# rhmes/point-cloud-compression

Hardware: AMD Instinct MI355X
Metric: points/sec compress+decompress (ModelNet40-shaped 8192 K=256) (higher is better)
Workload: dtype f32 (operands split into two scaled fp16 pieces of 22-23 bits together, three fp16-MFMA products per fp32 product, fp32 accumulate); 1 GPU; IPDAE K=256 d=16 L=7, 8192-pt CAD-like synthetic clouds (configs[1]); distinct_clouds_per_gpu=1024, points_per_cloud=8192, patches_per_cloud=64, octree_mode=reference, weights=seeded random, matmul=f16x2

## Files before the change

### point-cloud-compression_amd/csrc/rangecoder.hip

```cpp
#include "common.h"
#include "split_stream.h"
#include "entry_index.h"

struct BitWriter {
    uint8_t *buf;
    int cap, n;
    unsigned cache;
    int count;
    __device__ void bit(int b)
    {
        cache = (cache << 1) | (unsigned)(b & 1);
        if (++count == 8) {
            if (n < cap) buf[n] = (uint8_t)cache;
            ++n;
            count = 0; cache = 0;
        }
    }
    __device__ void bit_pending(int b, unsigned long long &pending)
    {
        bit(b);
        while (pending > 0) { bit(!b); --pending; }
    }
    __device__ void flush()
    {
        if (count > 0) {
            cache <<= (8 - count);
            if (n < cap) buf[n] = (uint8_t)cache;
            ++n;
            count = 0; cache = 0;
        }
    }
};

__device__ __forceinline__ int rc_row_bytes(int count, int stride) { return count < 0 ? 0 : (count > stride ? stride : count); }

__device__ __forceinline__ void rc_record(uint32_t *entry, unsigned low, unsigned high, unsigned long long bits, bool pending)
{
    entry[0] = low;
    entry[1] = high;
    entry[2] = (unsigned)(bits < 0x7FFFFFFFull ? bits : 0x7FFFFFFFull) | (pending ? PCCX_INDEX_FLAG : 0u);
}
__device__ __forceinline__ void rc_index_header(uint32_t *index, int nsym, int seg_sym)
{
    index[0] = 0x31495850u;
    index[1] = (unsigned)nsym;
    index[2] = (unsigned)seg_sym;
    index[3] = (unsigned)pccx_index_segments(nsym, seg_sym);
}

template <bool REC>
__device__ __forceinline__ void rc_encode_lane(const int32_t *__restrict__ cdf_int, const float *__restrict__ latent_q, int B, int nsym,
                                               int Lp, int sym_offset, uint8_t *__restrict__ out, int cap, int32_t *__restrict__ nbytes,
                                               int seg_sym, uint8_t *__restrict__ index, int idx_stride,
                                               const int32_t *__restrict__ nsym_of = nullptr)
{
    const int b = blockIdx.x * blockDim.x + threadIdx.x;
    if (b >= B) return;
    const int row = nsym;
    if (nsym_of) nsym = rc_row_bytes(nsym_of[b], row);
    uint32_t *entry = nullptr;
    if (REC) {
        entry = (uint32_t *)(index + (size_t)b * idx_stride);
        rc_index_header(entry, nsym, seg_sym);
        entry += PCCX_INDEX_HEADER_BYTES / 4;
    }
    BitWriter w{out + (size_t)b * cap, cap, 0, 0u, 0};
    unsigned low = 0u, high = 0xFFFFFFFFu;
    unsigned long long pending = 0;
    const int max_symbol = Lp - 2;
    const int32_t *c = cdf_int + (size_t)b * row * Lp;
    const float *q = latent_q + (size_t)b * row;
    int i = 0, stop = REC ? 0 : nsym;
    do {
    if (REC && i < nsym) {
        rc_record(entry, low, high, (unsigned long long)w.n * 8ull + (unsigned long long)w.count + pending, pending > 0);
        entry += PCCX_INDEX_ENTRY_BYTES / 4;
        stop = nsym - i < seg_sym ? nsym : i + seg_sym;
    }
    for (; i < stop; ++i, c += Lp) {
        int s = (int)q[i] + sym_offset;
        s = s < 0 ? 0 : (s > max_symbol ? max_symbol : s);
        const unsigned long long span = (unsigned long long)high - (unsigned long long)low + 1ull;
        const unsigned c_low = (unsigned)c[s] & 0xFFFFu;
        const unsigned c_high = s == max_symbol ? 0x10000u : ((unsigned)c[s + 1] & 0xFFFFu);
        high = (unsigned)((low - 1u) + (unsigned)((span * c_high) >> 16));
        low = (unsigned)(low + (unsigned)((span * c_low) >> 16));
        for (;;) {
            if (high < 0x80000000u) {
                w.bit_pending(0, pending);
                low <<= 1; high <<= 1; high |= 1u;
            } else if (low >= 0x80000000u) {
                w.bit_pending(1, pending);
                low <<= 1; high <<= 1; high |= 1u;
            } else if (low >= 0x40000000u && high < 0xC0000000u) {
                ++pending;
                low <<= 1; low &= 0x7FFFFFFFu;
                high <<= 1; high |= 0x80000001u;
            } else
                break;
        }
    }
    } while (REC && i < nsym);
    ++pending;
    if (low < 0x40000000u) w.bit_pending(0, pending);
    else w.bit_pending(1, pending);
    w.flush();
    nbytes[b] = w.n <= cap ? w.n : -w.n;
}

__global__ void range_encode_kernel(const int32_t *__restrict__ cdf_int, const float *__restrict__ latent_q, int B, int nsym,
                                    int Lp, int sym_offset, uint8_t *__restrict__ out, int cap, int32_t *__restrict__ nbytes)
{
    rc_encode_lane<false>(cdf_int, latent_q, B, nsym, Lp, sym_offset, out, cap, nbytes, 0, nullptr, 0);
}

__global__ void range_encode_indexed_kernel(const int32_t *__restrict__ cdf_int, const float *__restrict__ latent_q, int B, int nsym,
                                            int Lp, int sym_offset, uint8_t *__restrict__ out, int cap, int32_t *__restrict__ nbytes,
                                            int seg_sym, uint8_t *__restrict__ index, int idx_stride)
{
    rc_encode_lane<true>(cdf_int, latent_q, B, nsym, Lp, sym_offset, out, cap, nbytes, seg_sym, index, idx_stride);
}

template <bool REC>
__device__ __forceinline__ void rc_decode_lane(const int32_t *__restrict__ cdf_int, const uint8_t *__restrict__ in, int stride,
                                               const int32_t *__restrict__ nbytes, int B, int nsym, int Lp, int sym_offset,
                                               float *__restrict__ latent_q, int seg_sym, uint8_t *__restrict__ index, int idx_stride,
                                               const int32_t *__restrict__ nsym_of = nullptr)
{
    const int b = blockIdx.x * blockDim.x + threadIdx.x;
    if (b >= B) return;
    const int row = nsym;
    if (nsym_of) {
        nsym = rc_row_bytes(nsym_of[b], row);
        for (int i = nsym; i < row; ++i) latent_q[(size_t)b * row + i] = 0.f;
    }
    uint32_t *entry = nullptr;
    int next = 0;
    unsigned long long shifted = 0;
    bool under = false;
    if (REC) {
        entry = (uint32_t *)(index + (size_t)b * idx_stride);
        rc_index_header(entry, nsym, seg_sym);
        entry += PCCX_INDEX_HEADER_BYTES / 4;
    }
    const uint8_t *buf = in + (size_t)b * stride;
    const int nb = rc_row_bytes(nbytes[b], stride);
    int pos = 0, cached = 0;
    unsigned cache = 0;
    unsigned low = 0u, high = 0xFFFFFFFFu, value = 0u;
    auto get = [&]() {
        if (cached == 0) {
            if (pos >= nb) { value <<= 1; return; }
            cache = buf[pos++]; cached = 8;
        }
        value = (value << 1) | ((cache >> (cached - 1)) & 1u);
        --cached;
    };
    for (int i = 0; i < 32; ++i) get();
    const int max_symbol = Lp - 2;
    const int32_t *c = cdf_int + (size_t)b * row * Lp;
    for (int i = 0; i < nsym; ++i, c += Lp) {
        if (REC && i == next) {
            rc_record(entry, low, high, shifted, under);
            entry += PCCX_INDEX_ENTRY_BYTES / 4;
            next += seg_sym;
        }
        const unsigned long long span = (unsigned long long)high - (unsigned long long)low + 1ull;
        const unsigned count =
            (unsigned)((((unsigned long long)value - (unsigned long long)low + 1ull) * 0x10000ull - 1ull) / span) & 0xFFFFu;
        int left = 0, right = max_symbol + 1;
        while (left + 1 < right) {
            const int mid = (left + right) >> 1;
            if (((unsigned)c[mid] & 0xFFFFu) <= count) left = mid; else right = mid;
        }
        const int s = left;
        if (!REC || latent_q) latent_q[(size_t)b * row + i] = (float)(s - sym_offset);
        const unsigned c_low = (unsigned)c[s] & 0xFFFFu;
        const unsigned c_high = s == max_symbol ? 0x10000u : ((unsigned)c[s + 1] & 0xFFFFu);
        high = (unsigned)((low - 1u) + (unsigned)((span * c_high) >> 16));
        low = (unsigned)(low + (unsigned)((span * c_low) >> 16));
        for (;;) {
            if (low >= 0x80000000u || high < 0x80000000u) {
                low <<= 1; high <<= 1; high |= 1u; get();
                if (REC) ++shifted, under = false;
            } else if (low >= 0x40000000u && high < 0xC0000000u) {
                low <<= 1; low &= 0x7FFFFFFFu;
                high <<= 1; high |= 0x80000001u;
                value -= 0x40000000u;
                get();
                if (REC) ++shifted, under = true;
            } else
                break;
        }
    }
}

__global__ void range_decode_kernel(const int32_t *__restrict__ cdf_int, const uint8_t *__restrict__ in, int stride,
                                    const int32_t *__restrict__ nbytes, int B, int nsym, int Lp, int sym_offset,
                                    float *__restrict__ latent_q)
{
    rc_decode_lane<false>(cdf_int, in, stride, nbytes, B, nsym, Lp, sym_offset, latent_q, 0, nullptr, 0);
}

__global__ void range_index_build_kernel(const int32_t *__restrict__ cdf_int, const uint8_t *__restrict__ in, int stride,
                                         const int32_t *__restrict__ nbytes, int B, int nsym, int Lp, int sym_offset,
                                         float *__restrict__ latent_q, int seg_sym, uint8_t *__restrict__ index, int idx_stride)
{
    rc_decode_lane<true>(cdf_int, in, stride, nbytes, B, nsym, Lp, sym_offset, latent_q, seg_sym, index, idx_stride);
}

__global__ void range_encode_n_kernel(const int32_t *__restrict__ cdf_int, const float *__restrict__ latent_q, int B, int row,
                                      const int32_t *__restrict__ nsym_of, int Lp, int sym_offset, uint8_t *__restrict__ out, int cap,
                                      int32_t *__restrict__ nbytes)
{
    rc_encode_lane<false>(cdf_int, latent_q, B, row, Lp, sym_offset, out, cap, nbytes, 0, nullptr, 0, nsym_of);
}

__global__ void range_decode_n_kernel(const int32_t *__restrict__ cdf_int, const uint8_t *__restrict__ in, int stride,
                                      const int32_t *__restrict__ nbytes, int B, int row, const int32_t *__restrict__ nsym_of, int Lp,
                                      int sym_offset, float *__restrict__ latent_q)
{
    rc_decode_lane<false>(cdf_int, in, stride, nbytes, B, row, Lp, sym_offset, latent_q, 0, nullptr, 0, nsym_of);
}

#define RC_MAX_LDS_BYTES (60 * 1024)

__device__ __forceinline__ unsigned ones(int m) { return m >= 32 ? 0xFFFFFFFFu : ((1u << m) - 1u); }
__device__ __forceinline__ unsigned rc_uni(unsigned v) { return __builtin_amdgcn_readfirstlane(v); }
__device__ __forceinline__ unsigned rc_scale(unsigned span32, unsigned c) { return (unsigned)(((unsigned long long)span32 * c + c) >> 16); }

template <bool REC = false>
__device__ __forceinline__ void rc_encode_wave(unsigned char *smem, const int32_t *__restrict__ c, const float *__restrict__ q, int nsym,
                                               int Lp, int sym_offset, uint8_t *__restrict__ out, int cap, int32_t *__restrict__ nbytes,
                                               uint32_t *__restrict__ entry = nullptr, int seg_sym = 0)
{
    uint2 *sc = (uint2 *)smem;
    unsigned *sout = (unsigned *)(sc + nsym);
    const int lane = threadIdx.x;
    const int capw = (cap + 3) >> 2;
    const int max_symbol = Lp - 2;
    for (int i = lane; i < nsym; i += 64) {
        int s = (int)q[i] + sym_offset;
        s = s < 0 ? 0 : (s > max_symbol ? max_symbol : s);
        const int32_t *ci = c + (size_t)i * Lp;
        sc[i] = make_uint2((unsigned)ci[s] & 0xFFFFu, s == max_symbol ? 0x10000u : ((unsigned)ci[s + 1] & 0xFFFFu));
    }
    __syncthreads();
    unsigned low = 0u, high = 0xFFFFFFFFu;
    unsigned long long pending = 0, acc = 0;
    int na = 0, nw = 0;
    auto put = [&](unsigned v, int cnt) {
        acc = (acc << cnt) | (unsigned long long)v;
        na += cnt;
        if (na >= 32) {
            const unsigned w = (unsigned)(acc >> (na - 32));
            if (nw < capw && lane == 0) sout[nw] = __builtin_bswap32(w);
            ++nw;
            na -= 32;
        }
    };
    auto run = [&](int bit, unsigned long long cnt) {
        while (cnt > 0) {
            const int m = cnt > 32 ? 32 : (int)cnt;
            put(bit ? ones(m) : 0u, m);
            cnt -= m;
        }
    };
    int next = 0;
    uint2 nxt = lane < nsym ? sc[lane] : make_uint2(0u, 0x10000u);
    for (int i0 = 0; i0 < nsym; i0 += 64) {
        const uint2 cur = nxt;
        if (i0 + 64 + lane < nsym) nxt = sc[i0 + 64 + lane];
        const int cnt = nsym - i0 < 64 ? nsym - i0 : 64;
        for (int j = 0; j < cnt; ++j) {
            if (REC && i0 + j == next) {
                if (lane == 0) rc_record(entry, low, high, (unsigned long long)nw * 32ull + (unsigned long long)na + pending, pending > 0);
                entry += PCCX_INDEX_ENTRY_BYTES / 4;
                next += seg_sym;
            }
            const unsigned c_low = __builtin_amdgcn_readlane(cur.x, j), c_high = __builtin_amdgcn_readlane(cur.y, j);
            const unsigned span32 = high - low;
            high = (low - 1u) + rc_scale(span32, c_high);
            low = low + rc_scale(span32, c_low);
            const unsigned x = low ^ high;
            const int m = (int)x < 0 ? 0 : (x ? __clz(x) : 32);
            if (m > 0) {
                const unsigned top = (unsigned)(((unsigned long long)low << m) >> 32);
                if (pending == 0)
                    put(top, m);
                else {
                    const unsigned b0 = low >> 31;
                    put(b0, 1);
                    run(!b0, pending);
                    pending = 0;
                    if (m > 1) put(top & ones(m - 1), m - 1);
                }
                low = (unsigned)((unsigned long long)low << m);
                high = (unsigned)(((unsigned long long)high << m) | (unsigned long long)ones(m));
            }
            const unsigned t = (~low | high) << 1;
            const int k = t ? __clz(t) : 31;
            const unsigned fix = k ? 0x80000000u : 0u;
            low = (low << k) & ~fix;
            high = (high << k) | fix | ones(k);
            pending += k;
        }
    }
    ++pending;
    const int fb = low < 0x40000000u ? 0 : 1;
    put(fb, 1);
    run(!fb, pending);
    int n = nw * 4 + ((na + 7) >> 3);
    if (na > 0 && nw < capw && lane == 0) sout[nw] = __builtin_bswap32((unsigned)(acc << (32 - na)));
    if (lane == 0) *nbytes = n <= cap ? n : -n;
    __syncthreads();
    if (n > cap) n = cap;
    const uint8_t *sb = (const uint8_t *)sout;
    for (int i = lane; i < n; i += 64) out[i] = sb[i];
}

__global__ __launch_bounds__(64) void range_encode_wave_kernel(const int32_t *__restrict__ cdf_int, const float *__restrict__ latent_q,
                                                               int nsym, int Lp, int sym_offset, uint8_t *__restrict__ out, int cap,
                                                               int32_t *__restrict__ nbytes)
{
    extern __shared__ __attribute__((aligned(16))) unsigned char rc_smem[];
    const int b = blockIdx.x;
    rc_encode_wave(rc_smem, cdf_int + (size_t)b * nsym * Lp, latent_q + (size_t)b * nsym, nsym, Lp, sym_offset, out + (size_t)b * cap, cap,
                   nbytes + b);
}

__global__ __launch_bounds__(64) void range_encode_wave_n_kernel(const int32_t *__restrict__ cdf_int, const float *__restrict__ latent_q,
                                                                 int row, const int32_t *__restrict__ nsym_of, int Lp, int sym_offset,
                                                                 uint8_t *__restrict__ out, int cap, int32_t *__restrict__ nbytes)
{
    extern __shared__ __attribute__((aligned(16))) unsigned char rc_smem[];
    const int b = blockIdx.x;
    rc_encode_wave(rc_smem, cdf_int + (size_t)b * row * Lp, latent_q + (size_t)b * row, rc_row_bytes(nsym_of[b], row), Lp, sym_offset,
                   out + (size_t)b * cap, cap, nbytes + b);
}

template <bool INIT = false, bool REC = false>
__device__ __forceinline__ void rc_decode_wave(unsigned char *smem, const int32_t *__restrict__ c, const uint8_t *__restrict__ in, int stride,
                                               int nb, int nsym, int Lp, int sym_offset, float *__restrict__ q, unsigned low0 = 0u,
                                               unsigned high0 = 0xFFFFFFFFu, int skip = 0, bool under0 = false,
                                               uint32_t *__restrict__ entry = nullptr, int seg_sym = 0)
{
    const int ncdf = nsym * Lp;
    unsigned short *scdf = (unsigned short *)smem;
    unsigned *sin = (unsigned *)(smem + (((size_t)ncdf * 2 + 3) & ~(size_t)3));
    unsigned char *ssym = (unsigned char *)(sin + ((stride + 3) >> 2));
    const int lane = threadIdx.x;
    const int nwin = (nb + 3) >> 2;
    for (int i = lane; i < ncdf; i += 64) scdf[i] = (unsigned short)c[i];
    for (int i = lane; i < nwin * 4; i += 64) ((uint8_t *)sin)[i] = i < nb ? in[i] : (uint8_t)0;
    __syncthreads();
    auto word = [&](int p) -> unsigned { return p < nwin ? __builtin_bswap32(rc_uni(sin[p])) : 0u; };
    unsigned long long buf = 0;
    int have = 0, pos = 1;
    unsigned nxt = word(0);
    auto getbits = [&](int m) -> unsigned {
        if (have < m) {
            buf = (buf << 32) | (unsigned long long)nxt;
            have += 32;
            nxt = word(pos);
            ++pos;
        }
        have -= m;
        return (unsigned)(buf >> have) & ones(m);
    };
    unsigned low = 0u, high = 0xFFFFFFFFu;
    if (INIT) {
        low = low0, high = high0;
        getbits(skip & 7);
    }
    unsigned value = getbits(32);
    if (INIT) value ^= under0 ? 0x80000000u : 0u;
    unsigned long long shifted = 0;
    bool under = false;
    int next = 0;
    const int max_symbol = Lp - 2;
    const int G = 64 / Lp;
    unsigned cn = lane < G * Lp && lane < ncdf ? scdf[lane] : 0u;
    for (int i0 = 0; i0 < nsym; i0 += G) {
        const unsigned cv = cn;
        const int inext = (i0 + G) * Lp + lane;
        if (lane < G * Lp && inext < ncdf) cn = scdf[inext];
        const int cnt = nsym - i0 < G ? nsym - i0 : G;
        for (int j = 0; j < cnt; ++j) {
            if (REC && i0 + j == next) {
                if (lane == 0) rc_record(entry, low, high, shifted, under);
                entry += PCCX_INDEX_ENTRY_BYTES / 4;
                next += seg_sym;
            }
            const unsigned span32 = high - low, off = value - low;
            const unsigned t = rc_scale(span32, cv);
            const unsigned long long mask = __builtin_amdgcn_ballot_w64(t <= off) >> (j * Lp);
            const unsigned long long mr = (mask >> 1) & (~0ull >> (64 - max_symbol));
            int s = __popcll(mr);
            if ((mr + 1ull) & mr) {
                int left = 0, right = max_symbol + 1;
                while (left + 1 < right) {
                    const int mid = (left + right) >> 1;
                    if ((mask >> mid) & 1ull) left = mid; else right = mid;
                }
                s = left;
            }
            if (lane == 0) ssym[i0 + j] = (unsigned char)s;
            const unsigned t_low = __builtin_amdgcn_readlane(t, j * Lp + s);
            if (s != max_symbol) high = (low - 1u) + __builtin_amdgcn_readlane(t, j * Lp + s + 1);
            low = low + t_low;
            const unsigned x = low ^ high;
            const int m = (int)x < 0 ? 0 : (x ? __clz(x) : 32);
            low = (unsigned)((unsigned long long)low << m);
            high = (unsigned)(((unsigned long long)high << m) | (unsigned long long)ones(m));
            const unsigned tt = (~low | high) << 1;
            const int k = tt ? __clz(tt) : 31;
            const unsigned fix = k ? 0x80000000u : 0u;
            low = (low << k) & ~fix;
            high = (high << k) | fix | ones(k);
            const int n = m + k;
            if (REC) shifted += (unsigned)n, under = k > 0 || (m == 0 && under);
            if (n <= 32) {
                const unsigned nbits = getbits(n);
                value = ((unsigned)((unsigned long long)value << n) | nbits) ^ fix;
            } else {
                const unsigned v1 = (value << m) | getbits(m);
                value = ((v1 << k) ^ 0x80000000u) | getbits(k);
            }
        }
    }
    __syncthreads();
    if (REC && !q) return;
    for (int i = lane; i < nsym; i += 64) q[i] = (float)((int)ssym[i] - sym_offset);
}

__global__ __launch_bounds__(64) void range_decode_wave_kernel(const int32_t *__restrict__ cdf_int, const uint8_t *__restrict__ in,
                                                               int stride, const int32_t *__restrict__ nbytes, int nsym, int Lp,
                                                               int sym_offset, float *__restrict__ latent_q)
{
    extern __shared__ __attribute__((aligned(16))) unsigned char rc_smem[];
    const int b = blockIdx.x;
    const int nb = rc_row_bytes(nbytes[b], stride);
    rc_decode_wave(rc_smem, cdf_int + (size_t)b * nsym * Lp, in + (size_t)b * stride, stride, nb, nsym, Lp, sym_offset,
                   latent_q + (size_t)b * nsym);
}

__global__ __launch_bounds__(64) void range_decode_wave_n_kernel(const int32_t *__restrict__ cdf_int, const uint8_t *__restrict__ in,
                                                                 int stride, const int32_t *__restrict__ nbytes, int row,
                                                                 const int32_t *__restrict__ nsym_of, int Lp, int sym_offset,
                                                                 float *__restrict__ latent_q)
{
    extern __shared__ __attribute__((aligned(16))) unsigned char rc_smem[];
    const int b = blockIdx.x;
    const int nb = rc_row_bytes(nbytes[b], stride), ns = rc_row_bytes(nsym_of[b], row);
    float *q = latent_q + (size_t)b * row;
    rc_decode_wave(rc_smem, cdf_int + (size_t)b * row * Lp, in + (size_t)b * stride, stride, nb, ns, Lp, sym_offset, q);
    for (int i = ns + threadIdx.x; i < row; i += 64) q[i] = 0.f;
}

static size_t rc_encode_lds(int nsym, int cap) { return (size_t)nsym * 8 + (size_t)((cap + 3) / 4) * 4; }
static size_t rc_decode_lds(int nsym, int L, int stride)
{
    return (((size_t)nsym * (L + 1) * 2 + 3) & ~(size_t)3) + (size_t)((stride + 3) / 4) * 4 + (size_t)nsym;
}

extern "C" int pccx_range_coder_form(int decode, int nsym, int L, int cap_or_stride)
{
    if (nsym < 0 || L < 1 || cap_or_stride < 0) return 1;
    if (decode) return rc_decode_lds(nsym, L, cap_or_stride) <= RC_MAX_LDS_BYTES && L >= 2 && L + 1 <= 64 ? 0 : 1;
    return rc_encode_lds(nsym, cap_or_stride) <= RC_MAX_LDS_BYTES ? 0 : 1;
}

extern "C" int pccx_range_encode(const int32_t *cdf_int, const float *latent_q, int B, int nsym, int L, uint8_t *out, int cap,
                                 int32_t *nbytes, void *stream)
{
    if (B == 0) return PCCX_OK;
    PCCX_CHECK_ARG(cdf_int && latent_q && out && nbytes, "pccx_range_encode: null pointer");
    PCCX_CHECK_ARG(B >= 0 && nsym >= 0 && L >= 1 && cap >= 8, "pccx_range_encode: bad shape");
    const size_t lds = rc_encode_lds(nsym, cap);
    if (pccx_range_coder_form(0, nsym, L, cap) == 0) {
        hipLaunchKernelGGL(range_encode_wave_kernel, dim3(B), dim3(64), lds, (hipStream_t)stream, cdf_int, latent_q, nsym, L + 1,
                           L / 2, out, cap, nbytes);
        PCCX_CHECK_LAUNCH();
        return PCCX_OK;
    }
    hipLaunchKernelGGL(range_encode_kernel, dim3((B + 63) / 64), dim3(64), 0, (hipStream_t)stream, cdf_int, latent_q, B, nsym,
                       L + 1, L / 2, out, cap, nbytes);
    PCCX_CHECK_LAUNCH();
    return PCCX_OK;
}

extern "C" int pccx_range_decode(const int32_t *cdf_int, const uint8_t *in, int stride, const int32_t *nbytes, int B, int nsym,
                                 int L, float *latent_q, void *stream)
{
    if (B == 0) return PCCX_OK;
    PCCX_CHECK_ARG(cdf_int && in && nbytes && latent_q, "pccx_range_decode: null pointer");
    PCCX_CHECK_ARG(B >= 0 && nsym >= 0 && L >= 1 && stride >= 1, "pccx_range_decode: bad shape");
    const size_t lds = rc_decode_lds(nsym, L, stride);
    if (pccx_range_coder_form(1, nsym, L, stride) == 0) {
        hipLaunchKernelGGL(range_decode_wave_kernel, dim3(B), dim3(64), lds, (hipStream_t)stream, cdf_int, in, stride, nbytes, nsym,
                           L + 1, L / 2, latent_q);
        PCCX_CHECK_LAUNCH();
        return PCCX_OK;
    }
    hipLaunchKernelGGL(range_decode_kernel, dim3((B + 63) / 64), dim3(64), 0, (hipStream_t)stream, cdf_int, in, stride, nbytes,
                       B, nsym, L + 1, L / 2, latent_q);
    PCCX_CHECK_LAUNCH();
    return PCCX_OK;
}

extern "C" int pccx_range_encode_n(const int32_t *cdf_int, const float *latent_q, int B, int nsym, const int32_t *nsym_of, int L,
                                   uint8_t *out, int cap, int32_t *nbytes, void *stream)
{
    if (B == 0) return PCCX_OK;
    PCCX_CHECK_ARG(cdf_int && latent_q && nsym_of && out && nbytes, "pccx_range_encode_n: null pointer");
    PCCX_CHECK_ARG(B >= 0 && nsym >= 0 && L >= 1 && cap >= 8, "pccx_range_encode_n: bad shape");
    if (pccx_range_coder_form(0, nsym, L, cap) == 0)
        hipLaunchKernelGGL(range_encode_wave_n_kernel, dim3(B), dim3(64), rc_encode_lds(nsym, cap), (hipStream_t)stream, cdf_int, latent_q,
                           nsym, nsym_of, L + 1, L / 2, out, cap, nbytes);
    else
        hipLaunchKernelGGL(range_encode_n_kernel, dim3((B + 63) / 64), dim3(64), 0, (hipStream_t)stream, cdf_int, latent_q, B, nsym,
                           nsym_of, L + 1, L / 2, out, cap, nbytes);
    PCCX_CHECK_LAUNCH();
    return PCCX_OK;
}

extern "C" int pccx_range_decode_n(const int32_t *cdf_int, const uint8_t *in, int stride, const int32_t *nbytes, int B, int nsym,
                                   const int32_t *nsym_of, int L, float *latent_q, void *stream)
{
    if (B == 0) return PCCX_OK;
    PCCX_CHECK_ARG(cdf_int && in && nbytes && nsym_of && latent_q, "pccx_range_decode_n: null pointer");
    PCCX_CHECK_ARG(B >= 0 && nsym >= 0 && L >= 1 && stride >= 1, "pccx_range_decode_n: bad shape");
    if (pccx_range_coder_form(1, nsym, L, stride) == 0)
        hipLaunchKernelGGL(range_decode_wave_n_kernel, dim3(B), dim3(64), rc_decode_lds(nsym, L, stride), (hipStream_t)stream, cdf_int, in,
                           stride, nbytes, nsym, nsym_of, L + 1, L / 2, latent_q);
    else
        hipLaunchKernelGGL(range_decode_n_kernel, dim3((B + 63) / 64), dim3(64), 0, (hipStream_t)stream, cdf_int, in, stride, nbytes, B,
                           nsym, nsym_of, L + 1, L / 2, latent_q);
    PCCX_CHECK_LAUNCH();
    return PCCX_OK;
}

static int rc_split_segcap(int seg_sym) { return 2 * seg_sym + 16; }

extern "C" int pccx_range_split_max_seg_sym(int L)
{
    if (L < 2 || L > 63) return 0;
    int lo = 0, hi = RC_MAX_LDS_BYTES / 8;
    while (lo < hi) {
        const int mid = (lo + hi + 1) >> 1;
        if (rc_encode_lds(mid, rc_split_segcap(mid)) <= RC_MAX_LDS_BYTES && rc_decode_lds(mid, L, rc_split_segcap(mid)) <= RC_MAX_LDS_BYTES) lo = mid;
        else hi = mid - 1;
    }
    return lo;
}

extern "C" size_t pccx_range_split_workspace_bytes(int B, int nsym, int seg_sym)
{
    if (B <= 0 || nsym < 0 || seg_sym < 1) return 0;
    const size_t P = (size_t)pccx_split_segments(nsym, seg_sym);
    const size_t enc = (size_t)B * P * 4 + (size_t)B * P * (size_t)rc_split_segcap(seg_sym), dec = (size_t)B * (P + 1) * 4;
    return ((enc > dec ? enc : dec) + 15) & ~(size_t)15;
}

extern "C" int pccx_split_stream_check_host(const uint8_t *bytes, int64_t nbytes, int nsym, int seg_sym, int segcap)
{
    if (nsym < 0 || seg_sym < 1 || segcap < 0 || (!bytes && nbytes > 0)) return PCCX_SPLIT_BAD_FIELDS;
    return pccx_split_stream_check(bytes, nbytes, nsym, seg_sym, segcap, nullptr);
}

__global__ __launch_bounds__(64) void range_encode_split_kernel(const int32_t *__restrict__ cdf_int, const float *__restrict__ latent_q,
                                                                int nsym, int seg_sym, int P, int Lp, int sym_offset,
                                                                uint8_t *__restrict__ rows, int segcap, int32_t *__restrict__ counts)
{
    extern __shared__ __attribute__((aligned(16))) unsigned char rc_smem[];
    const int p = blockIdx.x, b = blockIdx.y;
    const int first = p * seg_sym;
    const int n = nsym - first < seg_sym ? nsym - first : seg_sym;
    const size_t row = (size_t)b * P + p;
    rc_encode_wave(rc_smem, cdf_int + ((size_t)b * nsym + first) * Lp, latent_q + (size_t)b * nsym + first, n, Lp, sym_offset,
                   rows + row * segcap, segcap, counts + row);
}

#define RC_PACK_THREADS 256
__global__ __launch_bounds__(RC_PACK_THREADS) void range_split_pack_kernel(const uint8_t *__restrict__ rows, const int32_t *__restrict__ counts,
                                                                          int nsym, int seg_sym, int P, int segcap,
                                                                          uint8_t *__restrict__ out, int cap, int32_t *__restrict__ nbytes)
{
    __shared__ int s_off[PCCX_SPLIT_MAX_SEGMENTS + 1];
    __shared__ long long s_part[RC_PACK_THREADS];
    __shared__ int s_bad;
    const int b = blockIdx.x, t = threadIdx.x;
    const int32_t *cnt = counts + (size_t)b * P;
    uint8_t *o = out + (size_t)b * cap;
    const int per = (P + RC_PACK_THREADS - 1) / RC_PACK_THREADS;
    const int p0 = t * per < P ? t * per : P, p1 = p0 + per < P ? p0 + per : P;
    if (t == 0) s_bad = 0;
    __syncthreads();
    long long sum = 0;
    int bad = 0;
    for (int p = p0; p < p1; ++p) {
        const int c = cnt[p];
        bad |= c < 0;
        sum += c < 0 ? -(long long)c : c;
    }
    s_part[t] = sum;
    if (bad) s_bad = 1;
    __syncthreads();
    const long long header = PCCX_SPLIT_HEADER_BYTES + 2ll * P;
    long long off = header;
    for (int i = 0; i < t; ++i) off += s_part[i];
    for (int p = p0; p < p1; ++p) {
        s_off[p] = (int)(off < cap ? off : cap);
        const int c = cnt[p];
        off += c < 0 ? -(long long)c : c;
    }
    if (t == RC_PACK_THREADS - 1) {
        s_off[P] = (int)(off < cap ? off : cap);
        if (blockIdx.y == 0) nbytes[b] = (off <= cap && !s_bad && off <= 0x7FFFFFFFll) ? (int)off : -(int)(off < 0x7FFFFFFFll ? off : 0x7FFFFFFFll);
    }
    __syncthreads();
    if (blockIdx.y == 0) {
        for (int i = t; i < header && i < cap; i += RC_PACK_THREADS) {
            unsigned v;
            if (i < 4) v = i == 0 ? 'P' : i == 1 ? 'X' : i == 2 ? 'S' : '1';
            else if (i < 8) v = ((unsigned)nsym >> (8 * (i - 4))) & 0xFFu;
            else if (i < 10) v = ((unsigned)seg_sym >> (8 * (i - 8))) & 0xFFu;
            else if (i < 12) v = 0u;
            else {
                const int c = cnt[(i - 12) >> 1];
                const unsigned len = (unsigned)(c < 0 ? (-(long long)c > 0xFFFF ? 0xFFFF : -c) : c);
                v = (len >> (8 * (i & 1))) & 0xFFu;
            }
            o[i] = (uint8_t)v;
        }
    }
    const int wave = t >> 6, lane = t & 63;
    for (int p = blockIdx.y * (RC_PACK_THREADS / 64) + wave; p < P; p += gridDim.y * (RC_PACK_THREADS / 64)) {
        const int c = cnt[p];
        int len = c < 0 ? segcap : c;
        len = len > segcap ? segcap : len;
        const int at = s_off[p];
        if (len > cap - at) len = cap - at;
        const uint8_t *src = rows + ((size_t)b * P + p) * segcap;
        for (int i = lane; i < len; i += 64) o[at + i] = src[i];
    }
}

__global__ __launch_bounds__(64) void range_split_check_kernel(const uint8_t *__restrict__ in, int stride, const int32_t *__restrict__ nbytes,
                                                               int B, int nsym, int seg_sym, int P, int segcap,
                                                               int32_t *__restrict__ status, int32_t *__restrict__ offsets)
{
    const int b = blockIdx.x * blockDim.x + threadIdx.x;
    if (b >= B) return;
    const int nb = rc_row_bytes(nbytes[b], stride);
    status[b] = pccx_split_stream_check(in + (size_t)b * stride, nb, nsym, seg_sym, segcap, offsets + (size_t)b * (P + 1));
}

struct RcSegment {
    int p, n, first;
};
template <bool LIST>
__device__ __forceinline__ RcSegment rc_segment(const int32_t *__restrict__ seg_idx, int nsym, int seg_sym, int P)
{
    RcSegment s;
    s.p = blockIdx.x;
    if (LIST) {
        const int p = (int)rc_uni((unsigned)seg_idx[blockIdx.x]);
        s.p = p < 0 ? 0 : (p > P - 1 ? P - 1 : p);
    }
    s.first = s.p * seg_sym;
    s.n = nsym - s.first < seg_sym ? nsym - s.first : seg_sym;
    return s;
}
template <bool LIST, class T>
__device__ __forceinline__ T *rc_segment_rows(T *base, const RcSegment &s, int nsym, int seg_sym, int width)
{
    const int j = blockIdx.x, b = blockIdx.y;
    return LIST ? base + (size_t)j * seg_sym * width : base + ((size_t)b * nsym + s.first) * width;
}

template <bool LIST>
__global__ __launch_bounds__(64) void range_decode_split_kernel(const int32_t *__restrict__ cdf_int, const uint8_t *__restrict__ in, int stride,
                                                                const int32_t *__restrict__ offsets, int nsym, int seg_sym, int P, int Lp,
                                                                int sym_offset, int segcap, float *__restrict__ latent_q,
                                                                const int32_t *__restrict__ seg_idx)
{
    extern __shared__ __attribute__((aligned(16))) unsigned char rc_smem[];
    const int b = blockIdx.y;
    const RcSegment s = rc_segment<LIST>(seg_idx, nsym, seg_sym, P);
    const int32_t *off = offsets + (size_t)b * (P + 1) + s.p;
    int at = (int)rc_uni((unsigned)off[0]), end = (int)rc_uni((unsigned)off[1]);
    at = at < 0 ? 0 : (at > stride ? stride : at);
    end = end < at ? at : (end > stride ? stride : end);
    const int nb = end - at > segcap ? segcap : end - at;
    rc_decode_wave(rc_smem, rc_segment_rows<LIST>(cdf_int, s, nsym, seg_sym, Lp), in + (size_t)b * stride + at, segcap, nb, s.n, Lp, sym_offset,
                   rc_segment_rows<LIST>(latent_q, s, nsym, seg_sym, 1));
}

static int rc_decode_split_launch(const int32_t *cdf_int, const uint8_t *in, int stride, const int32_t *nbytes, int B, int nsym, int seg_sym,
                                  int L, const int32_t *seg_idx, int n_waves, float *latent_q, int32_t *status, void *workspace,
                                  hipStream_t stream)
{
    const int P = (int)pccx_split_segments(nsym, seg_sym), segcap = rc_split_segcap(seg_sym);
    int32_t *offsets = (int32_t *)workspace;
    hipLaunchKernelGGL(range_split_check_kernel, dim3((B + 63) / 64), dim3(64), 0, stream, in, stride, nbytes, B, nsym, seg_sym, P, segcap,
                       status, offsets);
    PCCX_CHECK_LAUNCH();
    if (n_waves > 0) {
        const auto kernel = seg_idx ? range_decode_split_kernel<true> : range_decode_split_kernel<false>;
        hipLaunchKernelGGL(kernel, dim3(n_waves, B), dim3(64),
                           rc_decode_lds(seg_sym, L, segcap), stream, cdf_int, in, stride, offsets, nsym, seg_sym, P, L + 1, L / 2, segcap,
                           latent_q, seg_idx);
        PCCX_CHECK_LAUNCH();
    }
    return PCCX_OK;
}

static int rc_split_check_args(const char *who, int B, int nsym, int seg_sym, int L)
{
    PCCX_CHECK_ARG(B >= 0 && B <= 65535 && nsym >= 0 && seg_sym >= 1, "%s: bad shape (B=%d, nsym=%d, seg_sym=%d)", who, B, nsym, seg_sym);
    PCCX_CHECK_ARG(L >= 2 && L <= 63, "%s: L=%d; the wave kernels take 2 <= L <= 63", who, L);
    PCCX_CHECK_ARG(seg_sym <= pccx_range_split_max_seg_sym(L),
                   "%s: seg_sym=%d does not fit the %d bytes of LDS a segment is staged in; the largest seg_sym at L=%d is %d", who, seg_sym,
                   RC_MAX_LDS_BYTES, L, pccx_range_split_max_seg_sym(L));
    PCCX_CHECK_ARG(pccx_split_segments(nsym, seg_sym) <= PCCX_SPLIT_MAX_SEGMENTS, "%s: %lld segments; at most %d (nsym=%d, seg_sym=%d)", who,
                   (long long)pccx_split_segments(nsym, seg_sym), PCCX_SPLIT_MAX_SEGMENTS, nsym, seg_sym);
    return PCCX_OK;
}

extern "C" int pccx_range_encode_split(const int32_t *cdf_int, const float *latent_q, int B, int nsym, int seg_sym, int L, uint8_t *out,
                                       int cap, int32_t *nbytes, void *workspace, void *stream)
{
    if (B == 0) return PCCX_OK;
    const int rc = rc_split_check_args("pccx_range_encode_split", B, nsym, seg_sym, L);
    if (rc != PCCX_OK) return rc;
    const int P = (int)pccx_split_segments(nsym, seg_sym), segcap = rc_split_segcap(seg_sym);
    PCCX_CHECK_ARG(out && nbytes && (nsym == 0 || (cdf_int && latent_q && workspace)), "pccx_range_encode_split: null pointer");
    PCCX_CHECK_ARG(cap >= 8, "pccx_range_encode_split: bad shape (cap=%d)", cap);
    int32_t *counts = (int32_t *)workspace;
    uint8_t *rows = (uint8_t *)workspace + (size_t)B * P * 4;
    if (P > 0) {
        hipLaunchKernelGGL(range_encode_split_kernel, dim3(P, B), dim3(64), rc_encode_lds(seg_sym, segcap), (hipStream_t)stream, cdf_int,
                           latent_q, nsym, seg_sym, P, L + 1, L / 2, rows, segcap, counts);
        PCCX_CHECK_LAUNCH();
    }
    const int slices = P > 4 * 64 ? 64 : (P + 3) / 4 > 0 ? (P + 3) / 4 : 1;
    hipLaunchKernelGGL(range_split_pack_kernel, dim3(B, slices), dim3(RC_PACK_THREADS), 0, (hipStream_t)stream, rows, counts, nsym, seg_sym, P,
                       segcap, out, cap, nbytes);
    PCCX_CHECK_LAUNCH();
    return PCCX_OK;
}

extern "C" int pccx_range_decode_split(const int32_t *cdf_int, const uint8_t *in, int stride, const int32_t *nbytes, int B, int nsym,
                                       int seg_sym, int L, float *latent_q, int32_t *status, void *workspace, void *stream)
{
    if (B == 0) return PCCX_OK;
    const int rc = rc_split_check_args("pccx_range_decode_split", B, nsym, seg_sym, L);
    if (rc != PCCX_OK) return rc;
    PCCX_CHECK_ARG(in && nbytes && status && workspace && (nsym == 0 || (cdf_int && latent_q)), "pccx_range_decode_split: null pointer");
    PCCX_CHECK_ARG(stride >= 1, "pccx_range_decode_split: bad shape (stride=%d)", stride);
    return rc_decode_split_launch(cdf_int, in, stride, nbytes, B, nsym, seg_sym, L, nullptr, (int)pccx_split_segments(nsym, seg_sym), latent_q,
                                  status, workspace, (hipStream_t)stream);
}

extern "C" int pccx_range_decode_split_list(const int32_t *cdf_int, const uint8_t *in, int stride, const int32_t *nbytes, int nsym,
                                            int seg_sym, int L, const int32_t *seg_idx, int n_list, float *latent_q, int32_t *status,
                                            void *workspace, void *stream)
{
    const int rc = rc_split_check_args("pccx_range_decode_split_list", 1, nsym, seg_sym, L);
    if (rc != PCCX_OK) return rc;
    const int P = (int)pccx_split_segments(nsym, seg_sym);
    PCCX_CHECK_ARG(n_list >= 0 && n_list <= P, "pccx_range_decode_split_list: %d segments listed of %d", n_list, P);
    PCCX_CHECK_ARG(in && nbytes && status && workspace && (n_list == 0 || (cdf_int && latent_q && seg_idx)),
                   "pccx_range_decode_split_list: null pointer");
    PCCX_CHECK_ARG(stride >= 1, "pccx_range_decode_split_list: bad shape (stride=%d)", stride);
    return rc_decode_split_launch(cdf_int, in, stride, nbytes, 1, nsym, seg_sym, L, seg_idx, n_list, latent_q, status, workspace,
                                  (hipStream_t)stream);
}

static int rc_index_maxspan(int seg_sym) { return 8 * rc_split_segcap(seg_sym); }
static int rc_index_stage(int seg_sym) { return rc_split_segcap(seg_sym) + 8; }

extern "C" size_t pccx_range_index_bytes(int nsym, int seg_sym)
{
    if (nsym < 0 || seg_sym < 1) return 0;
    return (size_t)pccx_index_bytes(nsym, seg_sym);
}

extern "C" size_t pccx_range_index_workspace_bytes(int B, int nsym, int seg_sym)
{
    if (B <= 0 || nsym < 0 || seg_sym < 1) return 0;
    return (((size_t)B * (size_t)pccx_index_segments(nsym, seg_sym) * PCCX_INDEX_SEG_WORDS * 4) + 15) & ~(size_t)15;
}

extern "C" int pccx_entry_index_check_host(const uint8_t *index, int64_t idx_bytes, int64_t stream_bytes, int nsym, int seg_sym)
{
    if (nsym < 0 || seg_sym < 1 || seg_sym > (1 << 24) || idx_bytes < 0 || stream_bytes < 0 || stream_bytes > 0x7FFFFFFFll || (!index && idx_bytes > 0))
        return PCCX_INDEX_BAD_FIELDS;
    return pccx_entry_index_check(index, idx_bytes, stream_bytes, nsym, seg_sym, rc_index_maxspan(seg_sym), nullptr);
}

__global__ __launch_bounds__(64) void range_encode_indexed_wave_kernel(const int32_t *__restrict__ cdf_int, const float *__restrict__ latent_q,
                                                                       int nsym, int Lp, int sym_offset, uint8_t *__restrict__ out, int cap,
                                                                       int32_t *__restrict__ nbytes, int seg_sym, uint8_t *__restrict__ index,
                                                                       int idx_stride)
{
    extern __shared__ __attribute__((aligned(16))) unsigned char rc_smem[];
    const int b = blockIdx.x;
    uint32_t *side = (uint32_t *)(index + (size_t)b * idx_stride);
    if (threadIdx.x == 0) rc_index_header(side, nsym, seg_sym);
    rc_encode_wave<true>(rc_smem, cdf_int + (size_t)b * nsym * Lp, latent_q + (size_t)b * nsym, nsym, Lp, sym_offset, out + (size_t)b * cap,
                         cap, nbytes + b, side + PCCX_INDEX_HEADER_BYTES / 4, seg_sym);
}

__global__ __launch_bounds__(64) void range_index_build_wave_kernel(const int32_t *__restrict__ cdf_int, const uint8_t *__restrict__ in,
                                                                    int stride, const int32_t *__restrict__ nbytes, int nsym, int Lp,
                                                                    int sym_offset, float *__restrict__ latent_q, int seg_sym,
                                                                    uint8_t *__restrict__ index, int idx_stride)
{
    extern __shared__ __attribute__((aligned(16))) unsigned char rc_smem[];
    const int b = blockIdx.x;
    const int nb = rc_row_bytes(nbytes[b], stride);
    uint32_t *side = (uint32_t *)(index + (size_t)b * idx_stride);
    if (threadIdx.x == 0) rc_index_header(side, nsym, seg_sym);
    rc_decode_wave<false, true>(rc_smem, cdf_int + (size_t)b * nsym * Lp, in + (size_t)b * stride, stride, nb, nsym, Lp, sym_offset,
                                latent_q ? latent_q + (size_t)b * nsym : nullptr, 0u, 0xFFFFFFFFu, 0, false,
                                side + PCCX_INDEX_HEADER_BYTES / 4, seg_sym);
}

__global__ __launch_bounds__(64) void range_index_check_kernel(const uint8_t *__restrict__ index, int idx_stride, const int32_t *__restrict__ idx_nbytes,
                                                               int stride, const int32_t *__restrict__ nbytes, int B, int nsym, int seg_sym,
                                                               int P, int maxspan, int32_t *__restrict__ status, uint32_t *__restrict__ seg)
{
    const int b = blockIdx.x * blockDim.x + threadIdx.x;
    if (b >= B) return;
    const int nb = rc_row_bytes(nbytes[b], stride);
    const int ni = !idx_nbytes ? idx_stride : rc_row_bytes(idx_nbytes[b], idx_stride);
    status[b] = pccx_entry_index_check(index + (size_t)b * idx_stride, ni, nb, nsym, seg_sym, maxspan, seg + (size_t)b * P * PCCX_INDEX_SEG_WORDS);
}

__device__ __forceinline__ void rc_decode_entry(unsigned char *smem, const int32_t *__restrict__ c, const uint8_t *__restrict__ in, int nbrow,
                                                const uint32_t *__restrict__ seg, int stage, int n, int Lp, int sym_offset,
                                                float *__restrict__ q)
{
    const unsigned low = rc_uni(seg[0]), high = rc_uni(seg[1]), pf = rc_uni(seg[2]), end = rc_uni(seg[3]);
    const unsigned pos = pf & ~PCCX_INDEX_FLAG;
    int at = (int)(pos >> 3);
    const unsigned endb = (end >> 3) + ((end & 7u) ? 1u : 0u);
    int to = endb > (unsigned)nbrow ? nbrow : (int)endb;
    at = at > nbrow ? nbrow : at;
    to = to < at ? at : to;
    const int nb = to - at > stage ? stage : to - at;
    rc_decode_wave<true>(smem, c, in + at, stage, nb, n, Lp, sym_offset, q, low, high, (int)(pos & 7u), (pf & PCCX_INDEX_FLAG) != 0u);
}

template <bool LIST>
__global__ __launch_bounds__(64) void range_decode_indexed_kernel(const int32_t *__restrict__ cdf_int, const uint8_t *__restrict__ in, int stride,
                                                                  const int32_t *__restrict__ nbytes, const uint32_t *__restrict__ seg,
                                                                  int nsym, int seg_sym, int P, int Lp, int sym_offset, int stage,
                                                                  float *__restrict__ latent_q, const int32_t *__restrict__ seg_idx)
{
    extern __shared__ __attribute__((aligned(16))) unsigned char rc_smem[];
    const int b = blockIdx.y;
    const RcSegment s = rc_segment<LIST>(seg_idx, nsym, seg_sym, P);
    const int nbrow = rc_row_bytes((int)rc_uni((unsigned)nbytes[b]), stride);
    rc_decode_entry(rc_smem, rc_segment_rows<LIST>(cdf_int, s, nsym, seg_sym, Lp), in + (size_t)b * stride, nbrow,
                    seg + ((size_t)b * P + s.p) * PCCX_INDEX_SEG_WORDS, stage, s.n, Lp, sym_offset,
                    rc_segment_rows<LIST>(latent_q, s, nsym, seg_sym, 1));
}

static int rc_decode_indexed_launch(const int32_t *cdf_int, const uint8_t *in, int stride, const int32_t *nbytes, const uint8_t *index,
                                    int idx_stride, const int32_t *idx_nbytes, int B, int nsym, int seg_sym, int L, const int32_t *seg_idx,
                                    int n_waves, float *latent_q, int32_t *status, void *workspace, hipStream_t stream)
{
    const int P = (int)pccx_index_segments(nsym, seg_sym), stage = rc_index_stage(seg_sym);
    uint32_t *seg = (uint32_t *)workspace;
    hipLaunchKernelGGL(range_index_check_kernel, dim3((B + 63) / 64), dim3(64), 0, stream, index, idx_stride, idx_nbytes, stride, nbytes, B,
                       nsym, seg_sym, P, rc_index_maxspan(seg_sym), status, seg);
    PCCX_CHECK_LAUNCH();
    if (n_waves > 0) {
        const auto kernel = seg_idx ? range_decode_indexed_kernel<true> : range_decode_indexed_kernel<false>;
        hipLaunchKernelGGL(kernel, dim3(n_waves, B), dim3(64),
                           rc_decode_lds(seg_sym, L, stage), stream, cdf_int, in, stride, nbytes, seg, nsym, seg_sym, P, L + 1, L / 2, stage,
                           latent_q, seg_idx);
        PCCX_CHECK_LAUNCH();
    }
    return PCCX_OK;
}

static int rc_index_check_args(const char *who, int B, int nsym, int seg_sym, int L, int64_t stream_bytes)
{
    const int rc = rc_split_check_args(who, B, nsym, seg_sym, L);
    if (rc != PCCX_OK) return rc;
    PCCX_CHECK_ARG(stream_bytes >= 1 && stream_bytes <= (1 << 27), "%s: a stream row of %lld bytes; 1 .. 2^27 (bit positions are 31 bits wide)", who,
                   (long long)stream_bytes);
    return PCCX_OK;
}

extern "C" int pccx_range_encode_indexed(const int32_t *cdf_int, const float *latent_q, int B, int nsym, int seg_sym, int L, uint8_t *out,
                                         int cap, int32_t *nbytes, uint8_t *index, void *stream)
{
    if (B == 0) return PCCX_OK;
    const int rc = rc_index_check_args("pccx_range_encode_indexed", B, nsym, seg_sym, L, cap);
    if (rc != PCCX_OK) return rc;
    PCCX_CHECK_ARG(cdf_int && latent_q && out && nbytes && index, "pccx_range_encode_indexed: null pointer");
    PCCX_CHECK_ARG(cap >= 8 && ((uintptr_t)index & 3) == 0, "pccx_range_encode_indexed: bad shape (cap=%d) or an index that is not 4-byte aligned", cap);
    const int idx_stride = (int)pccx_index_bytes(nsym, seg_sym);
    if (pccx_range_coder_form(0, nsym, L, cap) == 0) {
        hipLaunchKernelGGL(range_encode_indexed_wave_kernel, dim3(B), dim3(64), rc_encode_lds(nsym, cap), (hipStream_t)stream, cdf_int, latent_q,
                           nsym, L + 1, L / 2, out, cap, nbytes, seg_sym, index, idx_stride);
        PCCX_CHECK_LAUNCH();
        return PCCX_OK;
    }
    hipLaunchKernelGGL(range_encode_indexed_kernel, dim3((B + 63) / 64), dim3(64), 0, (hipStream_t)stream, cdf_int, latent_q, B, nsym, L + 1,
                       L / 2, out, cap, nbytes, seg_sym, index, idx_stride);
    PCCX_CHECK_LAUNCH();
    return PCCX_OK;
}

extern "C" int pccx_range_index_build(const int32_t *cdf_int, const uint8_t *in, int stride, const int32_t *nbytes, int B, int nsym,
                                      int seg_sym, int L, uint8_t *index, float *latent_q, void *stream)
{
    if (B == 0) return PCCX_OK;
    const int rc = rc_index_check_args("pccx_range_index_build", B, nsym, seg_sym, L, stride);
    if (rc != PCCX_OK) return rc;
    PCCX_CHECK_ARG(cdf_int && in && nbytes && index, "pccx_range_index_build: null pointer");
    PCCX_CHECK_ARG(((uintptr_t)index & 3) == 0, "pccx_range_index_build: an index that is not 4-byte aligned");
    const int idx_stride = (int)pccx_index_bytes(nsym, seg_sym);
    if (pccx_range_coder_form(1, nsym, L, stride) == 0) {
        hipLaunchKernelGGL(range_index_build_wave_kernel, dim3(B), dim3(64), rc_decode_lds(nsym, L, stride), (hipStream_t)stream, cdf_int, in,
                           stride, nbytes, nsym, L + 1, L / 2, latent_q, seg_sym, index, idx_stride);
        PCCX_CHECK_LAUNCH();
        return PCCX_OK;
    }
    hipLaunchKernelGGL(range_index_build_kernel, dim3((B + 63) / 64), dim3(64), 0, (hipStream_t)stream, cdf_int, in, stride, nbytes, B, nsym,
                       L + 1, L / 2, latent_q, seg_sym, index, idx_stride);
    PCCX_CHECK_LAUNCH();
    return PCCX_OK;
}

extern "C" int pccx_range_decode_indexed(const int32_t *cdf_int, const uint8_t *in, int stride, const int32_t *nbytes, const uint8_t *index,
                                         int idx_stride, const int32_t *idx_nbytes, int B, int nsym, int seg_sym, int L, float *latent_q,
                                         int32_t *status, void *workspace, void *stream)
{
    if (B == 0) return PCCX_OK;
    const int rc = rc_index_check_args("pccx_range_decode_indexed", B, nsym, seg_sym, L, stride);
    if (rc != PCCX_OK) return rc;
    PCCX_CHECK_ARG(in && nbytes && index && status && workspace && (nsym == 0 || (cdf_int && latent_q)), "pccx_range_decode_indexed: null pointer");
    PCCX_CHECK_ARG(idx_stride >= 0, "pccx_range_decode_indexed: bad shape (idx_stride=%d)", idx_stride);
    return rc_decode_indexed_launch(cdf_int, in, stride, nbytes, index, idx_stride, idx_nbytes, B, nsym, seg_sym, L, nullptr,
                                    (int)pccx_index_segments(nsym, seg_sym), latent_q, status, workspace, (hipStream_t)stream);
}

extern "C" int pccx_range_decode_indexed_list(const int32_t *cdf_int, const uint8_t *in, int stride, const int32_t *nbytes,
                                              const uint8_t *index, int idx_bytes, int nsym, int seg_sym, int L, const int32_t *seg_idx,
                                              int n_list, float *latent_q, int32_t *status, void *workspace, void *stream)
{
    const int rc = rc_index_check_args("pccx_range_decode_indexed_list", 1, nsym, seg_sym, L, stride);
    if (rc != PCCX_OK) return rc;
    const int P = (int)pccx_index_segments(nsym, seg_sym);
    PCCX_CHECK_ARG(n_list >= 0 && n_list <= P, "pccx_range_decode_indexed_list: %d segments listed of %d", n_list, P);
    PCCX_CHECK_ARG(in && nbytes && index && status && workspace && (n_list == 0 || (cdf_int && latent_q && seg_idx)),
                   "pccx_range_decode_indexed_list: null pointer");
    PCCX_CHECK_ARG(idx_bytes >= 0, "pccx_range_decode_indexed_list: bad shape (idx_bytes=%d)", idx_bytes);
    return rc_decode_indexed_launch(cdf_int, in, stride, nbytes, index, idx_bytes, nullptr, 1, nsym, seg_sym, L, seg_idx, n_list, latent_q,
                                    status, workspace, (hipStream_t)stream);
}

__global__ void cdf_float_to_int_kernel(const float *__restrict__ cdf, int64_t n, int Lp, int32_t *__restrict__ out)
{
    const int64_t i = (int64_t)blockIdx.x * blockDim.x + threadIdx.x;
    if (i >= n) return;
    const int l = (int)(i % Lp);
    out[i] = ((int)rintf(__fmul_rn(cdf[i], (float)(65536 - (Lp - 1)))) + l) & 0xFFFF;
}

extern "C" int pccx_cdf_float_to_int(const float *cdf, int64_t nrows, int Lp, int32_t *cdf_int, void *stream)
{
    if (nrows == 0) return PCCX_OK;
    PCCX_CHECK_ARG(cdf && cdf_int, "pccx_cdf_float_to_int: null pointer");
    PCCX_CHECK_ARG(nrows > 0 && Lp >= 2 && Lp <= 65536, "pccx_cdf_float_to_int: bad shape");
    const int64_t n = nrows * Lp;
    hipLaunchKernelGGL(cdf_float_to_int_kernel, dim3((unsigned)((n + 255) / 256)), dim3(256), 0, (hipStream_t)stream, cdf, n, Lp, cdf_int);
    PCCX_CHECK_LAUNCH();
    return PCCX_OK;
}
```

Baseline: 1.097 billion points/s.

## Batch range-coder word and symbol writes via wave-register staging with writelane

The single-wave range encoder and decoder now collect output words and decoded symbols in a per-lane register using writelane, and flush them to LDS once every 64 entries instead of having lane 0 issue a scalar store on every step. The decoder prefetches input words into a register and reads them with readlane. Branches in the renormalisation are simplified so there are fewer conditionals per symbol. CDF staging and the final output or latent copies use wider vectorised loads and stores. The intent is to shorten the serial per-symbol critical path. The cost is more intricate buffering logic and edge cases at the flush boundaries.

```diff
diff --git a/point-cloud-compression_amd/csrc/rangecoder.hip b/point-cloud-compression_amd/csrc/rangecoder.hip
--- a/point-cloud-compression_amd/csrc/rangecoder.hip
+++ b/point-cloud-compression_amd/csrc/rangecoder.hip
@@ -225,8 +225,10 @@
 
 #define RC_MAX_LDS_BYTES (60 * 1024)
 
-__device__ __forceinline__ unsigned ones(int m) { return m >= 32 ? 0xFFFFFFFFu : ((1u << m) - 1u); }
+__device__ __forceinline__ unsigned ones(int m) { return ~(unsigned)(~0ull << m); }
 __device__ __forceinline__ unsigned rc_uni(unsigned v) { return __builtin_amdgcn_readfirstlane(v); }
+extern "C" __device__ int rc_llvm_writelane(int v, int lane, int old) __asm("llvm.amdgcn.writelane.i32");
+__device__ __forceinline__ unsigned rc_writelane(unsigned v, int lane, unsigned old) { return (unsigned)rc_llvm_writelane((int)v, lane, (int)old); }
 __device__ __forceinline__ unsigned rc_scale(unsigned span32, unsigned c) { return (unsigned)(((unsigned long long)span32 * c + c) >> 16); }
 
 template <bool REC = false>
@@ -239,24 +241,51 @@
     const int lane = threadIdx.x;
     const int capw = (cap + 3) >> 2;
     const int max_symbol = Lp - 2;
-    for (int i = lane; i < nsym; i += 64) {
-        int s = (int)q[i] + sym_offset;
-        s = s < 0 ? 0 : (s > max_symbol ? max_symbol : s);
-        const int32_t *ci = c + (size_t)i * Lp;
-        sc[i] = make_uint2((unsigned)ci[s] & 0xFFFFu, s == max_symbol ? 0x10000u : ((unsigned)ci[s + 1] & 0xFFFFu));
+    for (int i0 = 0; i0 < nsym; i0 += 256) {
+        int at[4], s[4];
+        unsigned lo[4], hi[4];
+#pragma unroll
+        for (int u = 0; u < 4; ++u) {
+            const int i = i0 + u * 64 + lane;
+            at[u] = i < nsym ? i : nsym - 1;
+            s[u] = (int)q[at[u]] + sym_offset;
+        }
+#pragma unroll
+        for (int u = 0; u < 4; ++u) {
+            s[u] = s[u] < 0 ? 0 : (s[u] > max_symbol ? max_symbol : s[u]);
+            const int32_t *ci = c + (size_t)at[u] * Lp;
+            lo[u] = (unsigned)ci[s[u]];
+            hi[u] = (unsigned)ci[s[u] + 1];
+        }
+#pragma unroll
+        for (int u = 0; u < 4; ++u) {
+            const int i = i0 + u * 64 + lane;
+            if (i < nsym) sc[i] = make_uint2(lo[u] & 0xFFFFu, s[u] == max_symbol ? 0x10000u : (hi[u] & 0xFFFFu));
+        }
     }
     __syncthreads();
     unsigned low = 0u, high = 0xFFFFFFFFu;
     unsigned long long pending = 0, acc = 0;
     int na = 0, nw = 0;
+    unsigned stage = 0u;
+    auto flush = [&](int base, int end) {
+        const int w = base + lane;
+        if ((unsigned)w < (unsigned)(end < capw ? end : capw)) sout[w] = __builtin_bswap32(stage);
+    };
+    auto word = [&](unsigned w) {
+        if ((nw & 63) == 0) {
+            __builtin_amdgcn_sched_barrier(0);
+            flush(nw - 64, nw);
+        }
+        stage = rc_writelane(w, nw & 63, stage);
+        ++nw;
+    };
     auto put = [&](unsigned v, int cnt) {
         acc = (acc << cnt) | (unsigned long long)v;
         na += cnt;
-        if (na >= 32) {
-            const unsigned w = (unsigned)(acc >> (na - 32));
-            if (nw < capw && lane == 0) sout[nw] = __builtin_bswap32(w);
-            ++nw;
+        if (__builtin_expect(na >= 32, 0)) {
             na -= 32;
+            word((unsigned)(acc >> na));
         }
     };
     auto run = [&](int bit, unsigned long long cnt) {
@@ -271,38 +300,41 @@
     for (int i0 = 0; i0 < nsym; i0 += 64) {
         const uint2 cur = nxt;
         if (i0 + 64 + lane < nsym) nxt = sc[i0 + 64 + lane];
-        const int cnt = nsym - i0 < 64 ? nsym - i0 : 64;
+        const int cnt = (int)rc_uni((unsigned)(nsym - i0 < 64 ? nsym - i0 : 64));
+        unsigned a_low = __builtin_amdgcn_readlane(cur.x, 0), a_high = __builtin_amdgcn_readlane(cur.y, 0);
         for (int j = 0; j < cnt; ++j) {
             if (REC && i0 + j == next) {
                 if (lane == 0) rc_record(entry, low, high, (unsigned long long)nw * 32ull + (unsigned long long)na + pending, pending > 0);
                 entry += PCCX_INDEX_ENTRY_BYTES / 4;
                 next += seg_sym;
             }
-            const unsigned c_low = __builtin_amdgcn_readlane(cur.x, j), c_high = __builtin_amdgcn_readlane(cur.y, j);
+            const unsigned c_low = a_low, c_high = a_high;
+            a_low = __builtin_amdgcn_readlane(cur.x, (j + 1) & 63), a_high = __builtin_amdgcn_readlane(cur.y, (j + 1) & 63);
             const unsigned span32 = high - low;
             high = (low - 1u) + rc_scale(span32, c_high);
             low = low + rc_scale(span32, c_low);
-            const unsigned x = low ^ high;
-            const int m = (int)x < 0 ? 0 : (x ? __clz(x) : 32);
-            if (m > 0) {
-                const unsigned top = (unsigned)(((unsigned long long)low << m) >> 32);
-                if (pending == 0)
-                    put(top, m);
-                else {
+            const int m = __clz(low ^ high);
+            const unsigned long long lm = (unsigned long long)low << m;
+            unsigned top = (unsigned)(lm >> 32);
+            int mb = m;
+            if (__builtin_expect(pending != 0, 0)) {
+                if (m > 0) {
                     const unsigned b0 = low >> 31;
                     put(b0, 1);
                     run(!b0, pending);
                     pending = 0;
-                    if (m > 1) put(top & ones(m - 1), m - 1);
+                    mb = m - 1;
+                    top &= ones(mb);
                 }
-                low = (unsigned)((unsigned long long)low << m);
-                high = (unsigned)(((unsigned long long)high << m) | (unsigned long long)ones(m));
             }
+            put(top, mb);
+            low = (unsigned)lm;
+            high = ~(unsigned)((unsigned long long)~high << m);
             const unsigned t = (~low | high) << 1;
-            const int k = t ? __clz(t) : 31;
+            const int k = __clz(t) < 31 ? __clz(t) : 31;
             const unsigned fix = k ? 0x80000000u : 0u;
             low = (low << k) & ~fix;
-            high = (high << k) | fix | ones(k);
+            high = ~(~high << k) | fix;
             pending += k;
         }
     }
@@ -311,12 +343,18 @@
     put(fb, 1);
     run(!fb, pending);
     int n = nw * 4 + ((na + 7) >> 3);
-    if (na > 0 && nw < capw && lane == 0) sout[nw] = __builtin_bswap32((unsigned)(acc << (32 - na)));
+    if (na > 0) word((unsigned)(acc << (32 - na)));
+    flush((nw - 1) & ~63, nw);
     if (lane == 0) *nbytes = n <= cap ? n : -n;
     __syncthreads();
     if (n > cap) n = cap;
     const uint8_t *sb = (const uint8_t *)sout;
-    for (int i = lane; i < n; i += 64) out[i] = sb[i];
+    int done = 0;
+    if (((uintptr_t)out & 3) == 0) {
+        done = n & ~3;
+        for (int i = lane; i < (done >> 2); i += 64) ((unsigned *)out)[i] = sout[i];
+    }
+    for (int i = done + lane; i < n; i += 64) out[i] = sb[i];
 }
 
 __global__ __launch_bounds__(64) void range_encode_wave_kernel(const int32_t *__restrict__ cdf_int, const float *__restrict__ latent_q,
@@ -351,19 +389,35 @@
     unsigned char *ssym = (unsigned char *)(sin + ((stride + 3) >> 2));
     const int lane = threadIdx.x;
     const int nwin = (nb + 3) >> 2;
-    for (int i = lane; i < ncdf; i += 64) scdf[i] = (unsigned short)c[i];
+    if (((uintptr_t)c & 15) == 0 && (ncdf & 3) == 0) {
+        const int4 *c4 = (const int4 *)c;
+        uint2 *s4 = (uint2 *)scdf;
+#pragma unroll 4
+        for (int i = lane; i < (ncdf >> 2); i += 64) {
+            const int4 v = c4[i];
+            s4[i] = make_uint2(((unsigned)v.x & 0xFFFFu) | ((unsigned)v.y << 16), ((unsigned)v.z & 0xFFFFu) | ((unsigned)v.w << 16));
+        }
+    } else
+        for (int i = lane; i < ncdf; i += 64) scdf[i] = (unsigned short)c[i];
     for (int i = lane; i < nwin * 4; i += 64) ((uint8_t *)sin)[i] = i < nb ? in[i] : (uint8_t)0;
     __syncthreads();
-    auto word = [&](int p) -> unsigned { return p < nwin ? __builtin_bswap32(rc_uni(sin[p])) : 0u; };
+    const int wlast = nwin > 0 ? nwin - 1 : 0;
+    auto raw = [&](int p0) -> unsigned { return sin[p0 + lane < wlast ? p0 + lane : wlast]; };
+    auto words = [&](unsigned r, int p0) -> unsigned { return p0 + lane < nwin ? __builtin_bswap32(r) : 0u; };
+    unsigned wcur = words(raw(0), 0), wraw = raw(64);
     unsigned long long buf = 0;
     int have = 0, pos = 1;
-    unsigned nxt = word(0);
+    unsigned nxt = __builtin_amdgcn_readlane(wcur, 0);
     auto getbits = [&](int m) -> unsigned {
-        if (have < m) {
+        if (__builtin_expect(have < m, 0)) {
             buf = (buf << 32) | (unsigned long long)nxt;
             have += 32;
-            nxt = word(pos);
+            nxt = __builtin_amdgcn_readlane(wcur, pos & 63);
             ++pos;
+            if ((pos & 63) == 0) {
+                wcur = words(wraw, pos);
+                wraw = raw(pos + 64);
+            }
         }
         have -= m;
         return (unsigned)(buf >> have) & ones(m);
@@ -381,11 +435,20 @@
     const int max_symbol = Lp - 2;
     const int G = 64 / Lp;
     unsigned cn = lane < G * Lp && lane < ncdf ? scdf[lane] : 0u;
+    unsigned sst = 0u;
+    int kept = 0;
+    auto store_symbols = [&](int end) {
+        const int i = end - 1 - ((end - 1 - lane) & 63);
+        if (i >= 0) ssym[i] = (unsigned char)sst;
+    };
     for (int i0 = 0; i0 < nsym; i0 += G) {
         const unsigned cv = cn;
         const int inext = (i0 + G) * Lp + lane;
         if (lane < G * Lp && inext < ncdf) cn = scdf[inext];
         const int cnt = nsym - i0 < G ? nsym - i0 : G;
+        const bool full = i0 + cnt - kept > 64;
+        if (full) store_symbols(i0);
+        kept = full ? i0 : kept;
         for (int j = 0; j < cnt; ++j) {
             if (REC && i0 + j == next) {
                 if (lane == 0) rc_record(entry, low, high, shifted, under);
@@ -405,33 +468,43 @@
                 }
                 s = left;
             }
-            if (lane == 0) ssym[i0 + j] = (unsigned char)s;
+            sst = rc_writelane((unsigned)s, (i0 + j) & 63, sst);
             const unsigned t_low = __builtin_amdgcn_readlane(t, j * Lp + s);
-            if (s != max_symbol) high = (low - 1u) + __builtin_amdgcn_readlane(t, j * Lp + s + 1);
+            const unsigned t_high = __builtin_amdgcn_readlane(t, j * Lp + s + 1);
+            high = s != max_symbol ? (low - 1u) + t_high : high;
             low = low + t_low;
-            const unsigned x = low ^ high;
-            const int m = (int)x < 0 ? 0 : (x ? __clz(x) : 32);
+            const int m = __clz(low ^ high);
             low = (unsigned)((unsigned long long)low << m);
-            high = (unsigned)(((unsigned long long)high << m) | (unsigned long long)ones(m));
+            high = ~(unsigned)((unsigned long long)~high << m);
             const unsigned tt = (~low | high) << 1;
-            const int k = tt ? __clz(tt) : 31;
+            const int k = __clz(tt) < 31 ? __clz(tt) : 31;
             const unsigned fix = k ? 0x80000000u : 0u;
             low = (low << k) & ~fix;
-            high = (high << k) | fix | ones(k);
-            const int n = m + k;
+            high = ~(~high << k) | fix;
+            int n = m + k;
             if (REC) shifted += (unsigned)n, under = k > 0 || (m == 0 && under);
-            if (n <= 32) {
-                const unsigned nbits = getbits(n);
-                value = ((unsigned)((unsigned long long)value << n) | nbits) ^ fix;
-            } else {
-                const unsigned v1 = (value << m) | getbits(m);
-                value = ((v1 << k) ^ 0x80000000u) | getbits(k);
+            if (__builtin_expect(n > 32, 0)) {
+                value = (value << m) | getbits(m);
+                n = k;
             }
-        }
-    }
+            const unsigned nbits = getbits(n);
+            value = ((unsigned)((unsigned long long)value << n) | nbits) ^ fix;
+        }
+    }
+    store_symbols(nsym);
     __syncthreads();
     if (REC && !q) return;
-    for (int i = lane; i < nsym; i += 64) q[i] = (float)((int)ssym[i] - sym_offset);
+    int done = 0;
+    if (((uintptr_t)q & 15) == 0) {
+        done = nsym & ~3;
+        const unsigned *s4 = (const unsigned *)ssym;
+        for (int i = lane; i < (done >> 2); i += 64) {
+            const unsigned v = s4[i];
+            ((float4 *)q)[i] = make_float4((float)((int)(v & 0xFFu) - sym_offset), (float)((int)((v >> 8) & 0xFFu) - sym_offset),
+                                           (float)((int)((v >> 16) & 0xFFu) - sym_offset), (float)((int)(v >> 24) - sym_offset));
+        }
+    }
+    for (int i = done + lane; i < nsym; i += 64) q[i] = (float)((int)ssym[i] - sym_offset);
 }
 
 __global__ __launch_bounds__(64) void range_decode_wave_kernel(const int32_t *__restrict__ cdf_int, const uint8_t *__restrict__ in,
```

Measured after the change: 1.083 billion points/s. 1.2% lower.
